# Windere/EAS-SNN

Measured on AMD Instinct MI355X. Metric: event-frames/sec (T=3) SYOLOX-S Gen1 304x240, higher is better.
Workload: dtype f32

## Files before the change

eas_snn_amd/csrc/pool.hip:

```cpp
#include "eas_common.h"

namespace {

constexpr int kMaxPlane = 1024;

struct SppGeom {
    int C, H, W, HW, ppb, r0, r1, r2;
    long long planes;
};

__device__ __forceinline__ bool better(float v, float bv) { return v > bv || v != v; }

__device__ __forceinline__ void spp_argmax(const float* plane, unsigned* rowarg, unsigned* amax, const SppGeom& g, int work) {
    const int rs[3] = {g.r0, g.r1, g.r2};
    const int rmax = max(g.r0, max(g.r1, g.r2));
    for (int idx = threadIdx.x; idx < work; idx += blockDim.x) {
        const int lp = idx / g.HW, i = idx - lp * g.HW, h = i / g.W, w = i - h * g.W;
        const float* row = plane + lp * g.HW + h * g.W;
        int best[3];
        float bv[3];
        bool have[3] = {false, false, false};
        const int b0 = w - rmax < 0 ? 0 : w - rmax, b1 = w + rmax >= g.W ? g.W - 1 : w + rmax;
        for (int b = b0; b <= b1; ++b) {
            const float v = row[b];
            const int d = b > w ? b - w : w - b;
#pragma unroll
            for (int j = 0; j < 3; ++j)
                if (d <= rs[j] && (!have[j] || better(v, bv[j]))) {
                    have[j] = true;
                    bv[j] = v;
                    best[j] = b;
                }
        }
        rowarg[idx] = (unsigned)best[0] | ((unsigned)best[1] << 10) | ((unsigned)best[2] << 20);
    }
    __syncthreads();
    for (int idx = threadIdx.x; idx < work; idx += blockDim.x) {
        const int lp = idx / g.HW, i = idx - lp * g.HW, h = i / g.W, w = i - h * g.W;
        const float* pl = plane + lp * g.HW;
        const unsigned* ra = rowarg + lp * g.HW;
        unsigned packed = 0;
#pragma unroll
        for (int j = 0; j < 3; ++j) {
            const int r = rs[j];
            const int a0 = h - r < 0 ? 0 : h - r, a1 = h + r >= g.H ? g.H - 1 : h + r;
            int best = a0 * g.W + (int)((ra[a0 * g.W + w] >> (10 * j)) & 1023u);
            float bv = pl[best];
            for (int a = a0 + 1; a <= a1; ++a) {
                const int q = a * g.W + (int)((ra[a * g.W + w] >> (10 * j)) & 1023u);
                const float v = pl[q];
                if (better(v, bv)) {
                    bv = v;
                    best = q;
                }
            }
            packed |= (unsigned)best << (10 * j);
        }
        amax[idx] = packed;
    }
}

__global__ __launch_bounds__(EAS_BLOCK) void spp_fwd_kernel(const float* __restrict__ x, float* __restrict__ out, SppGeom g) {
    extern __shared__ __align__(16) unsigned char spp_smem[];
    const int cap = g.ppb * g.HW;
    float* plane = reinterpret_cast<float*>(spp_smem);
    unsigned* rowarg = reinterpret_cast<unsigned*>(spp_smem) + cap;
    unsigned* amax = reinterpret_cast<unsigned*>(spp_smem) + 2 * cap;
    const long long p0 = (long long)blockIdx.x * g.ppb;
    const int np = (int)(g.planes - p0 < g.ppb ? g.planes - p0 : g.ppb);
    const int work = np * g.HW;
    const float* src = x + p0 * g.HW;
    for (int i = threadIdx.x; i < work; i += blockDim.x) plane[i] = src[i];
    __syncthreads();
    spp_argmax(plane, rowarg, amax, g, work);
    for (int idx = threadIdx.x; idx < work; idx += blockDim.x) {
        const int lp = idx / g.HW, i = idx - lp * g.HW;
        const long long pc = p0 + lp, n = pc / g.C, c = pc - n * g.C;
        float* dst = out + (n * 4 * g.C + c) * g.HW + i;
        const float* pl = plane + lp * g.HW;
        const unsigned pk = amax[idx];
        dst[0] = pl[i];
#pragma unroll
        for (int j = 0; j < 3; ++j) dst[(long long)(j + 1) * g.C * g.HW] = pl[(pk >> (10 * j)) & 1023u];
    }
}

template <bool XPL>
__global__ __launch_bounds__(EAS_BLOCK) void spp_bwd_kernel(const void* __restrict__ x_, const float* __restrict__ gout, float* __restrict__ gx,
                                                            SppGeom g) {
    extern __shared__ __align__(16) unsigned char spp_smem[];
    const int cap = g.ppb * g.HW;
    float* plane = reinterpret_cast<float*>(spp_smem);
    unsigned* rowarg = reinterpret_cast<unsigned*>(spp_smem) + cap;
    unsigned* amax = reinterpret_cast<unsigned*>(spp_smem) + 2 * cap;
    float* gp[3] = {plane + 3 * cap, plane + 4 * cap, plane + 5 * cap};
    float* tcol[3] = {plane + 6 * cap, plane + 7 * cap, plane + 8 * cap};
    unsigned* brow = reinterpret_cast<unsigned*>(spp_smem) + 9 * cap;
    const long long p0 = (long long)blockIdx.x * g.ppb;
    const int np = (int)(g.planes - p0 < g.ppb ? g.planes - p0 : g.ppb);
    const int work = np * g.HW;
    const float* src = reinterpret_cast<const float*>(x_) + p0 * g.HW;
    const __bf16* xp = reinterpret_cast<const __bf16*>(x_);
    for (int idx = threadIdx.x; idx < work; idx += blockDim.x) {
        const int lp = idx / g.HW, i = idx - lp * g.HW;
        const long long pc = p0 + lp, n = pc / g.C, c = pc - n * g.C;
        if constexpr (XPL) plane[idx] = (float)xp[((n * (g.C / 8) + c / 8) * g.HW + i) * 8 + (c & 7)];
        else plane[idx] = src[idx];
        const float* gsrc = gout + (n * 4 * g.C + c) * g.HW + i;
#pragma unroll
        for (int j = 0; j < 3; ++j) gp[j][idx] = gsrc[(long long)(j + 1) * g.C * g.HW];
    }
    __syncthreads();
    spp_argmax(plane, rowarg, amax, g, work);
    __syncthreads();
    for (int idx = threadIdx.x; idx < work; idx += blockDim.x) {
        const unsigned pk = amax[idx];
        brow[idx] = ((pk & 1023u) / g.W) | ((((pk >> 10) & 1023u) / g.W) << 10) | ((((pk >> 20) & 1023u) / g.W) << 20);
    }
    __syncthreads();
    const int rs[3] = {g.r0, g.r1, g.r2};
    for (int idx = threadIdx.x; idx < work; idx += blockDim.x) {
        const int lp = idx / g.HW, i = idx - lp * g.HW, h = i / g.W, b = i - h * g.W;
        const int base = lp * g.HW;
#pragma unroll
        for (int j = 0; j < 3; ++j) {
            const int r = rs[j];
            const int a0 = h - r < 0 ? 0 : h - r, a1 = h + r >= g.H ? g.H - 1 : h + r;
            float t = 0.f;
            for (int a = a0; a <= a1; ++a) {
                const int q = base + a * g.W + b;
                if ((int)((brow[q] >> (10 * j)) & 1023u) == h) t += gp[j][q];
            }
            tcol[j][idx] = t;
        }
    }
    __syncthreads();
    for (int idx = threadIdx.x; idx < work; idx += blockDim.x) {
        const int lp = idx / g.HW, i = idx - lp * g.HW, h = i / g.W, w = i - h * g.W;
        const long long pc = p0 + lp, n = pc / g.C, c = pc - n * g.C;
        const int rowbase = lp * g.HW + h * g.W;
        float s = gout[(n * 4 * g.C + c) * g.HW + i];
#pragma unroll
        for (int j = 0; j < 3; ++j) {
            const int r = rs[j];
            const int b0 = w - r < 0 ? 0 : w - r, b1 = w + r >= g.W ? g.W - 1 : w + r;
            for (int b = b0; b <= b1; ++b)
                if ((int)((rowarg[rowbase + b] >> (10 * j)) & 1023u) == w) s += tcol[j][rowbase + b];
        }
        gx[pc * g.HW + i] = s;
    }
}

typedef unsigned short u16x8 __attribute__((ext_vector_type(8)));

__global__ __launch_bounds__(EAS_BLOCK) void spp_planes_fwd_kernel(const u16x8* __restrict__ x, u16x8* __restrict__ out, SppGeom g) {
    extern __shared__ __align__(16) unsigned char spp_smem[];
    const int cap = g.ppb * g.HW;
    u16x8* map = reinterpret_cast<u16x8*>(spp_smem);
    u16x8* rowmax = map + cap;
    const long long p0 = (long long)blockIdx.x * g.ppb;
    const int np = (int)(g.planes - p0 < g.ppb ? g.planes - p0 : g.ppb);
    const int work = np * g.HW;
    const int G = g.C;
    for (int i = threadIdx.x; i < work; i += blockDim.x) map[i] = x[p0 * g.HW + i];
    __syncthreads();
    const int rs[3] = {g.r0, g.r1, g.r2};
    for (int idx = threadIdx.x; idx < work; idx += blockDim.x) {
        const int lp = idx / g.HW, i = idx - lp * g.HW, h = i / g.W, w = i - h * g.W;
        const u16x8* row = map + lp * g.HW + h * g.W;
#pragma unroll
        for (int j = 0; j < 3; ++j) {
            const int b0 = w - rs[j] < 0 ? 0 : w - rs[j], b1 = w + rs[j] >= g.W ? g.W - 1 : w + rs[j];
            u16x8 m = row[b0];
            for (int b = b0 + 1; b <= b1; ++b) m = __builtin_elementwise_max(m, row[b]);
            rowmax[j * cap + idx] = m;
        }
    }
    __syncthreads();
    for (int idx = threadIdx.x; idx < work; idx += blockDim.x) {
        const int lp = idx / g.HW, i = idx - lp * g.HW, h = i / g.W, w = i - h * g.W;
        const long long pg = p0 + lp, n = pg / G, grp = pg - n * G;
        u16x8* dst = out + (n * 4 * G + grp) * g.HW + i;
        dst[0] = map[idx];
#pragma unroll
        for (int j = 0; j < 3; ++j) {
            const int a0 = h - rs[j] < 0 ? 0 : h - rs[j], a1 = h + rs[j] >= g.H ? g.H - 1 : h + rs[j];
            const u16x8* col = rowmax + j * cap + lp * g.HW + w;
            u16x8 m = col[a0 * g.W];
            for (int a = a0 + 1; a <= a1; ++a) m = __builtin_elementwise_max(m, col[a * g.W]);
            dst[(long long)(j + 1) * G * g.HW] = m;
        }
    }
}

int make_geom(SppGeom& g, int64_t N, int C, int H, int W, int k0, int k1, int k2) {
    if (N <= 0 || C <= 0 || H <= 0 || W <= 0) return EAS_ERR_INVALID_ARG;
    if (H * W > kMaxPlane || !(k0 & 1) || !(k1 & 1) || !(k2 & 1) || k0 < 1 || k1 < 1 || k2 < 1 || N * C > 0x7fffffff) return EAS_ERR_UNSUPPORTED;
    g.C = C; g.H = H; g.W = W; g.HW = H * W;
    g.r0 = k0 / 2; g.r1 = k1 / 2; g.r2 = k2 / 2;
    g.planes = N * C;
    g.ppb = EAS_BLOCK / g.HW < 1 ? 1 : EAS_BLOCK / g.HW;
    return EAS_OK;
}

}

extern "C" {

int eas_spp_pool_fwd(const float* x, float* out, int64_t N, int C, int H, int W, int k0, int k1, int k2, eas_stream_t stream) {
    if (!x || !out) return EAS_ERR_INVALID_ARG;
    SppGeom g;
    if (int rc = make_geom(g, N, C, H, W, k0, k1, k2)) return rc;
    EAS_CLEAR_ERR();
    EAS_LAUNCH(spp_fwd_kernel, dim3((unsigned)((g.planes + g.ppb - 1) / g.ppb)), dim3(EAS_BLOCK), (size_t)3 * g.ppb * g.HW * 4, eas_s(stream), x, out, g);
    EAS_CHECK_LAUNCH();
    return EAS_OK;
}

int eas_spp_pool_bwd(const float* x, const float* grad_out, float* grad_x, int64_t N, int C, int H, int W, int k0, int k1, int k2,
                     eas_stream_t stream) {
    if (!x || !grad_out || !grad_x) return EAS_ERR_INVALID_ARG;
    SppGeom g;
    if (int rc = make_geom(g, N, C, H, W, k0, k1, k2)) return rc;
    EAS_CLEAR_ERR();
    EAS_LAUNCH(spp_bwd_kernel<false>, dim3((unsigned)((g.planes + g.ppb - 1) / g.ppb)), dim3(EAS_BLOCK), (size_t)10 * g.ppb * g.HW * 4, eas_s(stream),
               (const void*)x, grad_out, grad_x, g);
    EAS_CHECK_LAUNCH();
    return EAS_OK;
}

int eas_spp_pool_planes_fwd(const void* x_planes, void* out_planes, int64_t N, int C, int H, int W, int k0, int k1, int k2, eas_stream_t stream) {
    if (!x_planes || !out_planes) return EAS_ERR_INVALID_ARG;
    if (C % 8 != 0 || (((uintptr_t)x_planes | (uintptr_t)out_planes) & 15)) return EAS_ERR_UNSUPPORTED;
    SppGeom g;
    if (int rc = make_geom(g, N, C / 8, H, W, k0, k1, k2)) return rc;
    EAS_CLEAR_ERR();
    EAS_LAUNCH(spp_planes_fwd_kernel, dim3((unsigned)((g.planes + g.ppb - 1) / g.ppb)), dim3(EAS_BLOCK), (size_t)4 * g.ppb * g.HW * 16, eas_s(stream),
               (const u16x8*)x_planes, (u16x8*)out_planes, g);
    EAS_CHECK_LAUNCH();
    return EAS_OK;
}

int eas_spp_pool_planes_bwd(const void* x_planes, const float* grad_out, float* grad_x, int64_t N, int C, int H, int W, int k0, int k1, int k2,
                            eas_stream_t stream) {
    if (!x_planes || !grad_out || !grad_x) return EAS_ERR_INVALID_ARG;
    if (C % 8 != 0) return EAS_ERR_UNSUPPORTED;
    SppGeom g;
    if (int rc = make_geom(g, N, C, H, W, k0, k1, k2)) return rc;
    EAS_CLEAR_ERR();
    EAS_LAUNCH(spp_bwd_kernel<true>, dim3((unsigned)((g.planes + g.ppb - 1) / g.ppb)), dim3(EAS_BLOCK), (size_t)10 * g.ppb * g.HW * 4, eas_s(stream),
               x_planes, grad_out, grad_x, g);
    EAS_CHECK_LAUNCH();
    return EAS_OK;
}

}
```

Measured before the change: 3438.

## Add 8-channel packed SPP backward kernel with key-encoded argmax routing

Adds a new SPP max-pool backward kernel that works on 8-channel packed 16-bit planes. It computes separable row and column argmax by packing value and offset into 32-bit keys, then routes gradients back through the column and row passes in LDS. Per-thread items are templated, and the dynamic LDS limit is raised when the footprint needs it. The aim is to replace the scalar per-channel backward path with vectorized 8-wide processing, at the cost of a larger LDS footprint and therefore possibly lower occupancy.

Result: no change. 3466, median of 6 (+0.8%).

```diff
diff --git a/eas_snn_amd/csrc/pool.hip b/eas_snn_amd/csrc/pool.hip
--- a/eas_snn_amd/csrc/pool.hip
+++ b/eas_snn_amd/csrc/pool.hip
@@ -193,6 +193,141 @@
     }
 }
 
+constexpr int kSppBwdPixelBytes = 9 * 16;
+constexpr int kSppBias = 1024;
+constexpr size_t kSppBwdLdsDefault = 64 * 1024;
+constexpr size_t kSppBwdLdsMax = 160 * 1024;
+
+__device__ __forceinline__ void spp_key_max(unsigned (&key)[8], u16x8 v, unsigned inv) {
+    const uint4 p = __builtin_bit_cast(uint4, v);
+    const unsigned pair[4] = {p.x, p.y, p.z, p.w};
+#pragma unroll
+    for (int c = 0; c < 8; c += 2) {
+        key[c] = max(key[c], (pair[c / 2] << 16) | inv);
+        key[c + 1] = max(key[c + 1], (pair[c / 2] & 0xffff0000u) | inv);
+    }
+}
+__device__ __forceinline__ u16x8 spp_key_values(const unsigned (&key)[8]) {
+    u16x8 m;
+#pragma unroll
+    for (int c = 0; c < 8; ++c) m[c] = (unsigned short)(key[c] >> 16);
+    return m;
+}
+__device__ __forceinline__ u16x8 spp_key_codes(const unsigned (&key)[8]) {
+    u16x8 a;
+#pragma unroll
+    for (int c = 0; c < 8; ++c) a[c] = (unsigned short)(0xffffu - (key[c] & 0xffffu));
+    return a;
+}
+__device__ __forceinline__ void spp_add_where(float (&acc)[8], u16x8 rel, int code, float4 lo, float4 hi) {
+    const float v[8] = {lo.x, lo.y, lo.z, lo.w, hi.x, hi.y, hi.z, hi.w};
+#pragma unroll
+    for (int c = 0; c < 8; ++c) acc[c] = rel[c] == (unsigned short)code ? acc[c] + v[c] : acc[c];
+}
+
+template <int ITEMS>
+__global__ __launch_bounds__(EAS_BLOCK) void spp_planes_bwd_kernel(const u16x8* __restrict__ x, const float* __restrict__ gout,
+                                                                   float* __restrict__ gx, SppGeom g) {
+    extern __shared__ __align__(16) unsigned char spp_smem[];
+    const int cap = g.ppb * g.HW, HW = g.HW, W = g.W;
+    u16x8* map = reinterpret_cast<u16x8*>(spp_smem);
+    u16x8* rowmax = map + cap;
+    float4* gp = reinterpret_cast<float4*>(rowmax + cap);
+    float4* tcol = gp + 2 * cap;
+    u16x8* rowarg = reinterpret_cast<u16x8*>(tcol + 2 * cap);
+    u16x8* brow = rowarg + 2 * cap;
+    const int G = g.C;
+    const int p0 = (int)blockIdx.x * g.ppb;
+    const int np = (int)(g.planes - p0 < g.ppb ? g.planes - p0 : g.ppb);
+    const int work = np * HW;
+    const long long pool_stride = (long long)G * 8 * HW;
+    int idx[ITEMS], ph[ITEMS], pw[ITEMS];
+    long long gofs[ITEMS], xofs[ITEMS];
+    bool on[ITEMS];
+    float s[ITEMS][8];
+#pragma unroll
+    for (int k = 0; k < ITEMS; ++k) {
+        idx[k] = threadIdx.x + k * EAS_BLOCK;
+        on[k] = idx[k] < work;
+        if (on[k]) {
+            const int lp = idx[k] / HW, i = idx[k] - lp * HW, pg = p0 + lp, n = pg / G, grp = pg - n * G;
+            ph[k] = i / W;
+            pw[k] = i - ph[k] * W;
+            gofs[k] = ((long long)n * 4 * G + grp) * 8 * HW + i;
+            xofs[k] = (long long)pg * 8 * HW + i;
+            map[idx[k]] = x[(long long)p0 * HW + idx[k]];
+#pragma unroll
+            for (int c = 0; c < 8; ++c) s[k][c] = gout[gofs[k] + (long long)c * HW];
+        }
+    }
+    __syncthreads();
+#pragma unroll
+    for (int j = 0; j < 3; ++j) {
+        const int r = j == 0 ? g.r0 : (j == 1 ? g.r1 : g.r2);
+        u16x8* ra = rowarg + (j & 1) * cap;
+        float gv[ITEMS][8];
+#pragma unroll
+        for (int k = 0; k < ITEMS; ++k)
+            if (on[k]) {
+#pragma unroll
+                for (int c = 0; c < 8; ++c) gv[k][c] = gout[gofs[k] + (j + 1) * pool_stride + (long long)c * HW];
+            }
+#pragma unroll
+        for (int k = 0; k < ITEMS; ++k)
+            if (on[k]) {
+                const int w = pw[k], b0 = w - r < 0 ? 0 : w - r, b1 = w + r >= W ? W - 1 : w + r;
+                const u16x8* row = map + (idx[k] - w);
+                unsigned key[8] = {0, 0, 0, 0, 0, 0, 0, 0};
+                for (int b = b0; b <= b1; ++b) spp_key_max(key, row[b], 0xffffu - (unsigned)(b - w + kSppBias));
+                rowmax[idx[k]] = spp_key_values(key);
+                ra[idx[k]] = spp_key_codes(key);
+            }
+        __syncthreads();
+#pragma unroll
+        for (int k = 0; k < ITEMS; ++k)
+            if (on[k]) {
+                const int h = ph[k], a0 = h - r < 0 ? 0 : h - r, a1 = h + r >= g.H ? g.H - 1 : h + r;
+                const u16x8* col = rowmax + (idx[k] - h * W);
+                unsigned key[8] = {0, 0, 0, 0, 0, 0, 0, 0};
+                for (int a = a0; a <= a1; ++a) spp_key_max(key, col[a * W], 0xffffu - (unsigned)(a - h + kSppBias));
+                brow[idx[k]] = spp_key_codes(key);
+                gp[idx[k]] = make_float4(gv[k][0], gv[k][1], gv[k][2], gv[k][3]);
+                gp[cap + idx[k]] = make_float4(gv[k][4], gv[k][5], gv[k][6], gv[k][7]);
+            }
+        __syncthreads();
+#pragma unroll
+        for (int k = 0; k < ITEMS; ++k)
+            if (on[k]) {
+                const int h = ph[k], a0 = h - r < 0 ? 0 : h - r, a1 = h + r >= g.H ? g.H - 1 : h + r;
+                const int colbase = idx[k] - h * W;
+                float t[8] = {0.f, 0.f, 0.f, 0.f, 0.f, 0.f, 0.f, 0.f};
+                for (int a = a0; a <= a1; ++a) {
+                    const int q = colbase + a * W;
+                    spp_add_where(t, brow[q], h - a + kSppBias, gp[q], gp[cap + q]);
+                }
+                tcol[idx[k]] = make_float4(t[0], t[1], t[2], t[3]);
+                tcol[cap + idx[k]] = make_float4(t[4], t[5], t[6], t[7]);
+            }
+        __syncthreads();
+#pragma unroll
+        for (int k = 0; k < ITEMS; ++k)
+            if (on[k]) {
+                const int w = pw[k], b0 = w - r < 0 ? 0 : w - r, b1 = w + r >= W ? W - 1 : w + r;
+                const int rowbase = idx[k] - w;
+                for (int b = b0; b <= b1; ++b) {
+                    const int q = rowbase + b;
+                    spp_add_where(s[k], ra[q], w - b + kSppBias, tcol[q], tcol[cap + q]);
+                }
+            }
+    }
+#pragma unroll
+    for (int k = 0; k < ITEMS; ++k)
+        if (on[k]) {
+#pragma unroll
+            for (int c = 0; c < 8; ++c) gx[xofs[k] + (long long)c * HW] = s[k][c];
+        }
+}
+
 int make_geom(SppGeom& g, int64_t N, int C, int H, int W, int k0, int k1, int k2) {
     if (N <= 0 || C <= 0 || H <= 0 || W <= 0) return EAS_ERR_INVALID_ARG;
     if (H * W > kMaxPlane || !(k0 & 1) || !(k1 & 1) || !(k2 & 1) || k0 < 1 || k1 < 1 || k2 < 1 || N * C > 0x7fffffff) return EAS_ERR_UNSUPPORTED;
@@ -200,6 +335,27 @@
     g.r0 = k0 / 2; g.r1 = k1 / 2; g.r2 = k2 / 2;
     g.planes = N * C;
     g.ppb = EAS_BLOCK / g.HW < 1 ? 1 : EAS_BLOCK / g.HW;
+    return EAS_OK;
+}
+
+bool spp_planes_bwd_fits(const SppGeom& g, const void* x_planes) {
+    if ((uintptr_t)x_planes & 15) return false;
+    return (size_t)g.ppb * g.HW * kSppBwdPixelBytes <= kSppBwdLdsMax && g.ppb * g.HW <= 4 * EAS_BLOCK;
+}
+
+template <int ITEMS>
+int spp_planes_bwd_launch(const void* x_planes, const float* grad_out, float* grad_x, const SppGeom& g, eas_stream_t stream) {
+    const size_t lds = (size_t)g.ppb * g.HW * kSppBwdPixelBytes;
+    if (lds > kSppBwdLdsDefault) {
+        static bool raised = false;
+        if (!raised) {
+            if (hipFuncSetAttribute((const void*)spp_planes_bwd_kernel<ITEMS>, hipFuncAttributeMaxDynamicSharedMemorySize, (int)kSppBwdLdsMax) != hipSuccess)
+                return EAS_ERR_LAUNCH;
+            raised = true;
+        }
+    }
+    EAS_LAUNCH(spp_planes_bwd_kernel<ITEMS>, dim3((unsigned)((g.planes + g.ppb - 1) / g.ppb)), dim3(EAS_BLOCK), lds, eas_s(stream),
+               (const u16x8*)x_planes, grad_out, grad_x, g);
     return EAS_OK;
 }
 
@@ -248,6 +404,17 @@
     SppGeom g;
     if (int rc = make_geom(g, N, C, H, W, k0, k1, k2)) return rc;
     EAS_CLEAR_ERR();
+    SppGeom pg;
+    if (make_geom(pg, N, C / 8, H, W, k0, k1, k2) == EAS_OK && spp_planes_bwd_fits(pg, x_planes)) {
+        const int items = (pg.ppb * pg.HW + EAS_BLOCK - 1) / EAS_BLOCK;
+        int rc = items == 1   ? spp_planes_bwd_launch<1>(x_planes, grad_out, grad_x, pg, stream)
+                 : items == 2 ? spp_planes_bwd_launch<2>(x_planes, grad_out, grad_x, pg, stream)
+                 : items == 3 ? spp_planes_bwd_launch<3>(x_planes, grad_out, grad_x, pg, stream)
+                              : spp_planes_bwd_launch<4>(x_planes, grad_out, grad_x, pg, stream);
+        if (rc) return rc;
+        EAS_CHECK_LAUNCH();
+        return EAS_OK;
+    }
     EAS_LAUNCH(spp_bwd_kernel<true>, dim3((unsigned)((g.planes + g.ppb - 1) / g.ppb)), dim3(EAS_BLOCK), (size_t)10 * g.ppb * g.HW * 4, eas_s(stream),
                x_planes, grad_out, grad_x, g);
     EAS_CHECK_LAUNCH();
```
